# AlonKellner/hifi-gan

Hardware: NVIDIA B200
Metric: V1 audio samples/sec (higher is better)
Workload: dtype bf16

## Files before the change

hifi-gan_b200/csrc/hg_common.cuh:

```cuda
#pragma once

#include <cuda_runtime.h>
#include <cuda_bf16.h>
#include <cuda.h>
#include <stdint.h>
#include <stdio.h>

#define HG_OK 0
#define HG_ERR_INVALID (-1)
#define HG_ERR_CUDA (-2)
#define HG_ERR_UNSUPPORTED (-3)
#define HG_ERR_DRIVER (-4)

void hg_set_error(const char* fmt, ...);

#define HG_CHECK_CUDA(expr)                                                        \
  do {                                                                             \
    cudaError_t _e = (expr);                                                       \
    if (_e != cudaSuccess) {                                                       \
      hg_set_error("%s:%d: %s -> %s", __FILE__, __LINE__, #expr,                   \
                   cudaGetErrorString(_e));                                        \
      return HG_ERR_CUDA;                                                          \
    }                                                                              \
  } while (0)

#define HG_REQUIRE(cond, ...)                                                      \
  do {                                                                             \
    if (!(cond)) {                                                                 \
      hg_set_error(__VA_ARGS__);                                                   \
      return HG_ERR_INVALID;                                                       \
    }                                                                              \
  } while (0)

namespace hg {

#ifndef HG_SPIN_LIMIT
#define HG_SPIN_LIMIT (1u << 28)
#endif

__device__ __forceinline__ uint32_t smem_u32(const void* p) {
  return static_cast<uint32_t>(__cvta_generic_to_shared(p));
}

__device__ __forceinline__ bool elect_one() {
  uint32_t pred = 0;
  asm volatile(
      "{\n\t"
      ".reg .pred P;\n\t"
      "elect.sync _|P, 0xffffffff;\n\t"
      "selp.b32 %0, 1, 0, P;\n\t"
      "}\n"
      : "=r"(pred));
  return pred != 0;
}

__device__ __forceinline__ void mbar_init(uint64_t* bar, uint32_t count) {
  asm volatile("mbarrier.init.shared::cta.b64 [%0], %1;" ::"r"(smem_u32(bar)), "r"(count));
}
__device__ __forceinline__ void fence_mbar_init() {
  asm volatile("fence.mbarrier_init.release.cluster;" ::: "memory");
}
__device__ __forceinline__ void fence_proxy_async_smem() {
  asm volatile("fence.proxy.async.shared::cta;" ::: "memory");
}
__device__ __forceinline__ void mbar_arrive(uint64_t* bar) {
  asm volatile("mbarrier.arrive.shared::cta.b64 _, [%0];" ::"r"(smem_u32(bar)) : "memory");
}
__device__ __forceinline__ void mbar_arrive_expect_tx(uint64_t* bar, uint32_t bytes) {
  asm volatile("mbarrier.arrive.expect_tx.shared::cta.b64 _, [%0], %1;" ::"r"(smem_u32(bar)),
               "r"(bytes)
               : "memory");
}
__device__ __forceinline__ bool mbar_try_wait(uint64_t* bar, uint32_t parity) {
  uint32_t ok;
  asm volatile(
      "{\n\t"
      ".reg .pred P;\n\t"
      "mbarrier.try_wait.parity.shared::cta.b64 P, [%1], %2;\n\t"
      "selp.b32 %0, 1, 0, P;\n\t"
      "}\n"
      : "=r"(ok)
      : "r"(smem_u32(bar)), "r"(parity)
      : "memory");
  return ok != 0;
}
__device__ __forceinline__ void mbar_wait(uint64_t* bar, uint32_t parity) {
  uint32_t spins = 0;
  while (!mbar_try_wait(bar, parity)) {
    if (++spins > HG_SPIN_LIMIT) {
      printf("hg: mbarrier wait timed out (block %d thread %d)\n", (int)blockIdx.x, (int)threadIdx.x);
      __trap();
    }
  }
}

__device__ __forceinline__ void tma_prefetch_desc(const CUtensorMap* m) {
  asm volatile("prefetch.tensormap [%0];" ::"l"(reinterpret_cast<uint64_t>(m)) : "memory");
}
__device__ __forceinline__ void tma_load_3d(void* smem_dst, const CUtensorMap* m, uint64_t* bar,
                                            int32_t c0, int32_t c1, int32_t c2) {
  asm volatile(
      "cp.async.bulk.tensor.3d.shared::cluster.global.mbarrier::complete_tx::bytes"
      " [%0], [%1, {%3, %4, %5}], [%2];"
      :
      : "r"(smem_u32(smem_dst)), "l"(reinterpret_cast<uint64_t>(m)), "r"(smem_u32(bar)), "r"(c0),
        "r"(c1), "r"(c2)
      : "memory");
}

__device__ __forceinline__ void tc_fence_before() {
  asm volatile("tcgen05.fence::before_thread_sync;" ::: "memory");
}
__device__ __forceinline__ void tc_fence_after() {
  asm volatile("tcgen05.fence::after_thread_sync;" ::: "memory");
}
__device__ __forceinline__ void tmem_alloc(uint32_t* smem_result, uint32_t ncols) {
  asm volatile("tcgen05.alloc.cta_group::1.sync.aligned.shared::cta.b32 [%0], %1;" ::"r"(
                   smem_u32(smem_result)),
               "r"(ncols)
               : "memory");
  asm volatile("tcgen05.relinquish_alloc_permit.cta_group::1.sync.aligned;" ::: "memory");
}
__device__ __forceinline__ void tmem_dealloc(uint32_t taddr, uint32_t ncols) {
  asm volatile("tcgen05.dealloc.cta_group::1.sync.aligned.b32 %0, %1;" ::"r"(taddr), "r"(ncols)
               : "memory");
}
__device__ __forceinline__ void umma_bf16_ss_lo(uint32_t d_tmem, uint32_t a_lo, uint32_t b_lo,
                                                uint32_t desc_hi, uint32_t idesc, uint32_t accumulate) {
  asm volatile(
      "{\n\t"
      ".reg .pred p;\n\t"
      ".reg .b64 da, db;\n\t"
      "setp.ne.b32 p, %5, 0;\n\t"
      "mov.b64 da, {%1, %3};\n\t"
      "mov.b64 db, {%2, %3};\n\t"
      "tcgen05.mma.cta_group::1.kind::f16 [%0], da, db, %4, p;\n\t"
      "}\n"
      :
      : "r"(d_tmem), "r"(a_lo), "r"(b_lo), "r"(desc_hi), "r"(idesc), "r"(accumulate)
      : "memory");
}
__device__ __forceinline__ uint32_t cluster_ctarank() {
  uint32_t r;
  asm volatile("mov.u32 %0, %%cluster_ctarank;" : "=r"(r));
  return r;
}
__device__ __forceinline__ void cluster_sync_all() {
  asm volatile("barrier.cluster.arrive.release.aligned;" ::: "memory");
  asm volatile("barrier.cluster.wait.acquire.aligned;" ::: "memory");
}
__device__ __forceinline__ void mbar_arrive_remote(uint64_t* bar, uint32_t cta) {
  asm volatile(
      "{\n\t"
      ".reg .b32 remAddr32;\n\t"
      "mapa.shared::cluster.u32 remAddr32, %0, %1;\n\t"
      "mbarrier.arrive.shared::cluster.b64 _, [remAddr32];\n\t"
      "}\n"
      :
      : "r"(smem_u32(bar)), "r"(cta)
      : "memory");
}
__device__ __forceinline__ void tma_load_3d_2sm(void* smem_dst, const CUtensorMap* m, uint64_t* bar,
                                                int32_t c0, int32_t c1, int32_t c2) {
  asm volatile(
      "cp.async.bulk.tensor.3d.cta_group::2.shared::cluster.global.mbarrier::complete_tx::bytes"
      " [%0], [%1, {%3, %4, %5}], [%2];"
      :
      : "r"(smem_u32(smem_dst)), "l"(reinterpret_cast<uint64_t>(m)), "r"(smem_u32(bar) & 0xFEFFFFFFu),
        "r"(c0), "r"(c1), "r"(c2)
      : "memory");
}
__device__ __forceinline__ void tmem_alloc_2sm(uint32_t* smem_result, uint32_t ncols) {
  asm volatile("tcgen05.alloc.cta_group::2.sync.aligned.shared::cta.b32 [%0], %1;" ::"r"(
                   smem_u32(smem_result)),
               "r"(ncols)
               : "memory");
  asm volatile("tcgen05.relinquish_alloc_permit.cta_group::2.sync.aligned;" ::: "memory");
}
__device__ __forceinline__ void tmem_dealloc_2sm(uint32_t taddr, uint32_t ncols) {
  asm volatile("tcgen05.dealloc.cta_group::2.sync.aligned.b32 %0, %1;" ::"r"(taddr), "r"(ncols)
               : "memory");
}
__device__ __forceinline__ void umma_bf16_ss_lo_2sm(uint32_t d_tmem, uint32_t a_lo, uint32_t b_lo,
                                                    uint32_t desc_hi, uint32_t idesc, uint32_t accumulate) {
  asm volatile(
      "{\n\t"
      ".reg .pred p;\n\t"
      ".reg .b64 da, db;\n\t"
      "setp.ne.b32 p, %5, 0;\n\t"
      "mov.b64 da, {%1, %3};\n\t"
      "mov.b64 db, {%2, %3};\n\t"
      "tcgen05.mma.cta_group::2.kind::f16 [%0], da, db, %4, p;\n\t"
      "}\n"
      :
      : "r"(d_tmem), "r"(a_lo), "r"(b_lo), "r"(desc_hi), "r"(idesc), "r"(accumulate)
      : "memory");
}
__device__ __forceinline__ void umma_commit_2sm(uint64_t* bar) {
  asm volatile(
      "tcgen05.commit.cta_group::2.mbarrier::arrive::one.shared::cluster.multicast::cluster.b64 [%0], %1;"
      :
      : "r"(smem_u32(bar)), "h"(static_cast<uint16_t>(3))
      : "memory");
}

__device__ __forceinline__ uint32_t umma_desc_lo(uint32_t saddr) {
  return ((saddr & 0x3FFFFu) >> 4) | (1u << 16);
}
__device__ __forceinline__ uint32_t umma_desc_hi(uint32_t sbo_bytes, uint32_t layout_type) {
  return ((sbo_bytes >> 4) & 0x3FFFu) | (1u << 14) | ((layout_type & 7u) << 29);
}
__device__ __forceinline__ void umma_commit(uint64_t* bar) {
  asm volatile("tcgen05.commit.cta_group::1.mbarrier::arrive::one.shared::cluster.b64 [%0];" ::"r"(
                   smem_u32(bar))
               : "memory");
}
__device__ __forceinline__ void tmem_ld_wait() {
  asm volatile("tcgen05.wait::ld.sync.aligned;" ::: "memory");
}


__host__ __device__ constexpr uint32_t umma_idesc_bf16(uint32_t M, uint32_t N) {
  return (1u << 4) | (1u << 7) | (1u << 10) | ((N >> 3) << 17) | ((M >> 4) << 24);
}

__device__ __forceinline__ float lrelu(float v, float slope) { return v > 0.f ? v : v * slope; }

__device__ __forceinline__ uint32_t pack_bf16x2(float lo, float hi) {
  __nv_bfloat162 h = __floats2bfloat162_rn(lo, hi);
  return *reinterpret_cast<uint32_t*>(&h);
}
__device__ __forceinline__ float2 unpack_bf16x2(uint32_t w) {
  __nv_bfloat162 h = *reinterpret_cast<__nv_bfloat162*>(&w);
  return __bfloat1622float2(h);
}

struct U8 {
  uint32_t v[8];
};

__device__ __forceinline__ U8 ldg256(const void* p) {
  U8 r;
  asm volatile("ld.global.nc.L1::no_allocate.v8.b32 {%0,%1,%2,%3,%4,%5,%6,%7}, [%8];"
               : "=r"(r.v[0]), "=r"(r.v[1]), "=r"(r.v[2]), "=r"(r.v[3]), "=r"(r.v[4]), "=r"(r.v[5]),
                 "=r"(r.v[6]), "=r"(r.v[7])
               : "l"(p));
  return r;
}
__device__ __forceinline__ void stg256(void* p, const U8& r) {
  asm volatile("st.global.v8.b32 [%0], {%1,%2,%3,%4,%5,%6,%7,%8};" ::"l"(p), "r"(r.v[0]),
               "r"(r.v[1]), "r"(r.v[2]), "r"(r.v[3]), "r"(r.v[4]), "r"(r.v[5]), "r"(r.v[6]),
               "r"(r.v[7])
               : "memory");
}
__device__ __forceinline__ void tmem_ld_32x16(uint32_t taddr, uint32_t (&v)[16]) {
  asm volatile(
      "tcgen05.ld.sync.aligned.32x32b.x16.b32 "
      "{%0, %1, %2, %3, %4, %5, %6, %7, %8, %9, %10, %11, %12, %13, %14, %15}, [%16];"
      : "=r"(v[0]), "=r"(v[1]), "=r"(v[2]), "=r"(v[3]), "=r"(v[4]), "=r"(v[5]), "=r"(v[6]),
        "=r"(v[7]), "=r"(v[8]), "=r"(v[9]), "=r"(v[10]), "=r"(v[11]), "=r"(v[12]), "=r"(v[13]),
        "=r"(v[14]), "=r"(v[15])
      : "r"(taddr)
      : "memory");
}
__device__ __forceinline__ void add_bf16x16(float (&v)[16], const U8& r) {
#pragma unroll
  for (int i = 0; i < 8; ++i) {
    const float2 f = unpack_bf16x2(r.v[i]);
    v[2 * i] += f.x;
    v[2 * i + 1] += f.y;
  }
}
__device__ __forceinline__ void add_bf16x16_unlrelu(float (&v)[16], const U8& r, float inv_slope) {
#pragma unroll
  for (int i = 0; i < 8; ++i) {
    const float2 f = unpack_bf16x2(r.v[i]);
    v[2 * i] += fminf(f.x, f.x * inv_slope);
    v[2 * i + 1] += fminf(f.y, f.y * inv_slope);
  }
}



template <int N>
__device__ __forceinline__ float warp_colsum(float (&v)[N], int lane, int& col) {
  int off = 16;
  col = 0;
#pragma unroll
  for (int w = N / 2; w >= 1; w >>= 1) {
    const bool hi = (lane & off) != 0;
#pragma unroll
    for (int i = 0; i < w; ++i) {
      const float send = hi ? v[i] : v[i + w];
      const float keep = hi ? v[i + w] : v[i];
      v[i] = keep + __shfl_xor_sync(0xffffffffu, send, off);
    }
    if (hi) col += w;
    off >>= 1;
  }
#pragma unroll
  for (int o = 16; o >= 1; o >>= 1)
    if (o <= off) v[0] += __shfl_xor_sync(0xffffffffu, v[0], o);
  return v[0];
}

struct PerDeviceOnce {
  size_t done[64] = {};
  bool need(size_t want = 1) {
    int d = 0;
    if (cudaGetDevice(&d) != cudaSuccess || d < 0 || d >= 64) return true;
    if (done[d] >= want) return false;
    done[d] = want;
    return true;
  }
};
}

int hg_encode_tmap_bf16_3d(CUtensorMap* out, const void* base, uint64_t d0, uint64_t d1, uint64_t d2,
                           uint64_t stride1_bytes, uint64_t stride2_bytes, uint32_t box0,
                           uint32_t box1, uint32_t box2, int swizzle_bytes);
```

hifi-gan_b200/csrc/hg_resblock_pair.cu:

```cuda
#include "hg_common.cuh"

#include <atomic>

#include "../../include/hifigan_b200.h"

extern std::atomic<int64_t> g_hg_launches;

namespace {

constexpr int kM = 128;
constexpr int kXformWarps = 4;
__host__ __device__ constexpr int epi_halves(int c) { return c == 64 ? 2 : 1; }
__host__ __device__ constexpr int pair_threads(int c) { return 64 + (kXformWarps + 8 * epi_halves(c)) * 32; }
constexpr int kMaxXSlots = 4;

struct PairArgs {
  int batch, t, c;
  int ktaps, dil1;
  int single;
  int subs;
  int r_out;
  int pad1, pad2;
  int a_rows;
  int x_boxes, x_box_rows;
  int tiles_t, num_tiles;
  int x_slots;
  uint32_t x_slot_bytes, t1_slot_bytes, w_bytes;
  const __nv_bfloat16* x;
  const float* b1;
  const float* b2;
  const __nv_bfloat16* res1;
  const __nv_bfloat16* res2;
  float scale, in_slope, out_slope;
  __nv_bfloat16* out_raw;
  __nv_bfloat16* out_act;
  const int* item_len;
  int item_mul;
  float x_inv;
};

struct PairBarriers {
  uint64_t x_full[kMaxXSlots], x_ready[kMaxXSlots], x_empty[kMaxXSlots];
  uint64_t w_full;
  uint64_t acc1_full[2], acc1_empty[2], t1_full[2], t1_empty[2], acc2_full[2], acc2_empty[2];
  uint32_t tmem_base;
  uint32_t pad;
  __align__(16) float b1[64];
  __align__(16) float b2[64];
};

__device__ __forceinline__ uint32_t lrelu_bf16x2(uint32_t w, __nv_bfloat162 slope2) {
  __nv_bfloat162 v = *reinterpret_cast<__nv_bfloat162*>(&w);
  v = __hmax2(v, __hmul2(v, slope2));
  return *reinterpret_cast<uint32_t*>(&v);
}

template <int C, bool kSingle, bool kMrf, bool kActIn>
__global__ void __launch_bounds__(pair_threads(C), 1)
resblock_pair_kernel(const __grid_constant__ CUtensorMap tm_x, const __grid_constant__ CUtensorMap tm_w1,
                     const __grid_constant__ CUtensorMap tm_w2, const PairArgs p) {
  constexpr uint32_t kRowBytes = C * 2;
  constexpr uint32_t kLayout = (C == 64) ? 2u : 4u;
  constexpr uint32_t kSbo = 8 * kRowBytes;
  constexpr uint32_t kTapBytes = C * kRowBytes;
  constexpr int kChunksPerRow = kRowBytes / 16;
  constexpr int kHalves = epi_halves(C);
  constexpr int kRoleWarps = 4 * kHalves;
  constexpr int kThreads = pair_threads(C);

  extern __shared__ uint8_t smem_raw[];
  uint8_t* smem = reinterpret_cast<uint8_t*>((reinterpret_cast<uintptr_t>(smem_raw) + 1023) &
                                             ~static_cast<uintptr_t>(1023));
  uint8_t* x_buf = smem;
  uint8_t* t1_buf = x_buf + p.x_slots * p.x_slot_bytes;
  uint8_t* w1_buf = t1_buf + 2 * p.t1_slot_bytes;
  uint8_t* w2_buf = w1_buf + p.w_bytes;
  PairBarriers* bars = reinterpret_cast<PairBarriers*>(w1_buf + (kSingle ? 1 : 2) * p.w_bytes);

  const int warp = threadIdx.x >> 5;
  const int lane = threadIdx.x & 31;
  const int S = p.subs;
  const uint32_t acc_cols = static_cast<uint32_t>(S) * C;
  const uint32_t tmem_cols = 4 * acc_cols <= 128 ? 128u : 4 * acc_cols <= 256 ? 256u : 512u;

  if (warp == 0 && lane == 0) {
    hg::tma_prefetch_desc(&tm_x);
    hg::tma_prefetch_desc(&tm_w1);
    hg::tma_prefetch_desc(&tm_w2);
  }
  if (warp == 1) {
    if (lane == 0) {
      for (int i = 0; i < kMaxXSlots; ++i) {
        hg::mbar_init(&bars->x_full[i], 1);
        hg::mbar_init(&bars->x_ready[i], kXformWarps);
        hg::mbar_init(&bars->x_empty[i], 1);
      }
      hg::mbar_init(&bars->w_full, 1);
      for (int i = 0; i < 2; ++i) {
        hg::mbar_init(&bars->acc1_full[i], 1);
        hg::mbar_init(&bars->acc1_empty[i], kRoleWarps);
        hg::mbar_init(&bars->t1_full[i], kRoleWarps);
        hg::mbar_init(&bars->t1_empty[i], 1);
        hg::mbar_init(&bars->acc2_full[i], 1);
        hg::mbar_init(&bars->acc2_empty[i], kRoleWarps);
      }
      hg::fence_mbar_init();
    }
    __syncwarp();
    hg::tmem_alloc(&bars->tmem_base, tmem_cols);
  }
  if (threadIdx.x < C) {
    bars->b1[threadIdx.x] = p.b1[threadIdx.x];
    bars->b2[threadIdx.x] = p.b2[threadIdx.x];
  }
  for (uint32_t i = threadIdx.x * 16; i < 2 * p.t1_slot_bytes; i += kThreads * 16)
    *reinterpret_cast<uint4*>(t1_buf + i) = make_uint4(0, 0, 0, 0);
  hg::fence_proxy_async_smem();
  hg::tc_fence_before();
  __syncthreads();
  hg::tc_fence_after();
  const uint32_t tmem_base = *reinterpret_cast<volatile uint32_t*>(&bars->tmem_base);
  const int n_local = (p.num_tiles - static_cast<int>(blockIdx.x) + static_cast<int>(gridDim.x) - 1) /
                      static_cast<int>(gridDim.x);

  if (warp == 0) {
    if (lane == 0) {
      hg::mbar_arrive_expect_tx(&bars->w_full, (kSingle ? 1 : 2) * p.w_bytes);
      hg::tma_load_3d(w1_buf, &tm_w1, &bars->w_full, 0, 0, 0);
      if (!kSingle) hg::tma_load_3d(w2_buf, &tm_w2, &bars->w_full, 0, 0, 0);
      const uint32_t box_bytes = static_cast<uint32_t>(p.x_box_rows) * kRowBytes;
      int tt = blockIdx.x % p.tiles_t, b = blockIdx.x / p.tiles_t;
      const int tt_step = gridDim.x % p.tiles_t, b_step = gridDim.x / p.tiles_t;
      uint32_t slot = 0, phase = 0;
      for (int i = 0; i < n_local; ++i) {
        hg::mbar_wait(&bars->x_empty[slot], phase ^ 1u);
        hg::mbar_arrive_expect_tx(&bars->x_full[slot], box_bytes * p.x_boxes);
        for (int bx = 0; bx < p.x_boxes; ++bx)
          hg::tma_load_3d(x_buf + slot * p.x_slot_bytes + bx * box_bytes, &tm_x, &bars->x_full[slot], 0,
                          tt * p.r_out - p.pad2 - p.pad1 + bx * p.x_box_rows, b);
        if (++slot == static_cast<uint32_t>(p.x_slots)) { slot = 0; phase ^= 1u; }
        tt += tt_step; b += b_step;
        if (tt >= p.tiles_t) { tt -= p.tiles_t; ++b; }
      }
    }
    __syncwarp();
  } else if (warp == 1) {
    constexpr uint32_t idesc = hg::umma_idesc_bf16(kM, C);
    constexpr uint32_t kTapLo = kTapBytes >> 4;
    const uint32_t desc_hi = hg::umma_desc_hi(kSbo, kLayout);
    const uint32_t w1_lo = hg::umma_desc_lo(hg::smem_u32(w1_buf));
    const uint32_t w2_lo = hg::umma_desc_lo(hg::smem_u32(w2_buf));
    const uint32_t x_tap_step = static_cast<uint32_t>(p.dil1) * (kRowBytes >> 4);
    hg::mbar_wait(&bars->w_full, 0);
    hg::tc_fence_after();
    auto issue = [&](uint32_t d, uint32_t a_lo, uint32_t w_lo, uint32_t a_step) {
      uint32_t accumulate = 0;
      for (int j = 0; j < p.ktaps; ++j) {
#pragma unroll
        for (int kk = 0; kk < C / 16; ++kk) {
          hg::umma_bf16_ss_lo(d, a_lo + kk * 2, w_lo + kk * 2, desc_hi, idesc, accumulate);
          accumulate = 1;
        }
        a_lo += a_step;
        w_lo += kTapLo;
      }
    };
    uint32_t x_slot = 0, x_phase = 0;
    auto conv1 = [&](int i) {
      const uint32_t slot = x_slot, a = i & 1u, ph = (i >> 1) & 1u;
      hg::mbar_wait(&bars->x_ready[slot], x_phase);
      if (++x_slot == static_cast<uint32_t>(p.x_slots)) { x_slot = 0; x_phase ^= 1u; }
      hg::mbar_wait(&bars->acc1_empty[a], ph ^ 1u);
      hg::tc_fence_after();
      if (hg::elect_one()) {
        const uint32_t x_lo = hg::umma_desc_lo(hg::smem_u32(x_buf + slot * p.x_slot_bytes));
        for (int m = 0; m < S; ++m)
          issue(tmem_base + a * acc_cols + m * C, x_lo + m * (kM * (kRowBytes >> 4)), w1_lo, x_tap_step);
        hg::umma_commit(&bars->x_empty[slot]);
        hg::umma_commit(&bars->acc1_full[a]);
      }
      __syncwarp();
    };
    auto conv2 = [&](int i) {
      const uint32_t a = i & 1u, ph = (i >> 1) & 1u;
      hg::mbar_wait(&bars->t1_full[a], ph);
      hg::mbar_wait(&bars->acc2_empty[a], ph ^ 1u);
      hg::tc_fence_after();
      if (hg::elect_one()) {
        const uint32_t t_lo = hg::umma_desc_lo(hg::smem_u32(t1_buf + a * p.t1_slot_bytes));
        for (int m = 0; m < S; ++m)
          issue(tmem_base + 2 * acc_cols + a * acc_cols + m * C, t_lo + m * (kM * (kRowBytes >> 4)), w2_lo,
                kRowBytes >> 4);
        hg::umma_commit(&bars->t1_empty[a]);
        hg::umma_commit(&bars->acc2_full[a]);
      }
      __syncwarp();
    };
    if (kSingle) {
      for (int i = 0; i < n_local; ++i) conv1(i);
    } else {
      if (n_local > 0) conv1(0);
      for (int i = 0; i < n_local; ++i) {
        if (i + 1 < n_local) conv1(i + 1);
        conv2(i);
      }
    }
  } else if (warp < 2 + kXformWarps) {
    const int tid = (warp - 2) * 32 + lane;
    const __nv_bfloat162 slope2 = __float2bfloat162_rn(p.in_slope);
    const int n_chunks = p.a_rows * kChunksPerRow;
    uint32_t slot = 0, phase = 0;
    for (int i = 0; i < n_local; ++i) {
      hg::mbar_wait(&bars->x_full[slot], phase);
      if (!kActIn) {
        uint4* xs = reinterpret_cast<uint4*>(x_buf + slot * p.x_slot_bytes);
        for (int q = tid; q < n_chunks; q += kXformWarps * 32) {
          uint4 v = xs[q];
          v.x = lrelu_bf16x2(v.x, slope2); v.y = lrelu_bf16x2(v.y, slope2);
          v.z = lrelu_bf16x2(v.z, slope2); v.w = lrelu_bf16x2(v.w, slope2);
          xs[q] = v;
        }
        hg::fence_proxy_async_smem();
      }
      __syncwarp();
      if (lane == 0) hg::mbar_arrive(&bars->x_ready[slot]);
      if (++slot == static_cast<uint32_t>(p.x_slots)) { slot = 0; phase ^= 1u; }
    }
  } else {
    const int ew = warp - (2 + kXformWarps);
    const int quarter = warp & 3;
    const int half = (ew >> 2) % kHalves;
    const int row = quarter * 32 + lane;
    const uint32_t lane_base = static_cast<uint32_t>(quarter * 32) << 16;
    constexpr int kG = C / (16 * kHalves);
    const int col0 = half * (C / kHalves);

    if (ew < kRoleWarps) {
      const float* bias = bars->b1;
      const uint32_t swz = (C == 64) ? (row & 7) : ((row >> 1) & 3);
      int tt = blockIdx.x % p.tiles_t;
      int bb = blockIdx.x / p.tiles_t;
      const int tt_step = gridDim.x % p.tiles_t, b_step = gridDim.x / p.tiles_t;
      for (int i = 0; i < (kSingle ? 0 : n_local); ++i) {
        const uint32_t a = i & 1u, ph = (i >> 1) & 1u;
        hg::mbar_wait(&bars->acc1_full[a], ph);
        hg::mbar_wait(&bars->t1_empty[a], ph ^ 1u);
        hg::tc_fence_after();
        const int t_item = (kMrf && p.item_len) ? min(p.t, __ldg(p.item_len + bb) * p.item_mul) : p.t;
        for (int m = 0; m < S; ++m) {
          const int grow = m * kM + row;
          const int time = tt * p.r_out - p.pad2 + grow;
          const bool inside = time >= 0 && time < t_item;
          uint8_t* trow = t1_buf + a * p.t1_slot_bytes + static_cast<uint32_t>(grow) * kRowBytes;
#pragma unroll
          for (int g = 0; g < kG; ++g) {
            uint32_t raw[16];
            hg::tmem_ld_32x16(tmem_base + lane_base + a * acc_cols + m * C + col0 + g * 16, raw);
            hg::tmem_ld_wait();
            if (g == kG - 1 && m == S - 1) {
              hg::tc_fence_before();
              __syncwarp();
              if (lane == 0) hg::mbar_arrive(&bars->acc1_empty[a]);
            }
            uint32_t o[8];
#pragma unroll
            for (int q = 0; q < 4; ++q) {
              const float4 bq = *reinterpret_cast<const float4*>(bias + col0 + g * 16 + 4 * q);
              const float v0 = hg::lrelu(__uint_as_float(raw[4 * q]) + bq.x, p.in_slope);
              const float v1 = hg::lrelu(__uint_as_float(raw[4 * q + 1]) + bq.y, p.in_slope);
              const float v2 = hg::lrelu(__uint_as_float(raw[4 * q + 2]) + bq.z, p.in_slope);
              const float v3 = hg::lrelu(__uint_as_float(raw[4 * q + 3]) + bq.w, p.in_slope);
              o[2 * q] = inside ? hg::pack_bf16x2(v0, v1) : 0u;
              o[2 * q + 1] = inside ? hg::pack_bf16x2(v2, v3) : 0u;
            }
            const uint32_t chunk = (col0 >> 3) + g * 2;
            *reinterpret_cast<uint4*>(trow + ((chunk ^ swz) << 4)) = make_uint4(o[0], o[1], o[2], o[3]);
            *reinterpret_cast<uint4*>(trow + (((chunk + 1) ^ swz) << 4)) = make_uint4(o[4], o[5], o[6], o[7]);
          }
        }
        hg::fence_proxy_async_smem();
        __syncwarp();
        if (lane == 0) hg::mbar_arrive(&bars->t1_full[a]);
        tt += tt_step; bb += b_step;
        if (tt >= p.tiles_t) { tt -= p.tiles_t; ++bb; }
      }
    } else {
      const float* bias = kSingle ? bars->b1 : bars->b2;
      uint64_t* full_bar = kSingle ? bars->acc1_full : bars->acc2_full;
      uint64_t* empty_bar = kSingle ? bars->acc1_empty : bars->acc2_empty;
      const uint32_t acc_base = kSingle ? 0u : 2 * acc_cols;
      int n_tt = blockIdx.x % p.tiles_t, n_b = blockIdx.x / p.tiles_t, n_m = 0;
      const int tt_step = gridDim.x % p.tiles_t, b_step = gridDim.x / p.tiles_t;
      auto next_unit_off = [&](bool& valid, bool& keep) -> size_t {
        const int grow = n_m * kM + row;
        const int time = n_tt * p.r_out + grow;
        valid = grow < p.r_out && time < p.t;
        keep = !kMrf || !p.item_len || time < __ldg(p.item_len + n_b) * p.item_mul;
        const size_t o = (static_cast<size_t>(n_b) * p.t + (valid ? time : 0)) * C + col0;
        if (++n_m == S) {
          n_m = 0;
          n_tt += tt_step; n_b += b_step;
          if (n_tt >= p.tiles_t) { n_tt -= p.tiles_t; ++n_b; }
        }
        return o;
      };
      hg::U8 rcur[kG], rnext[kG];
      bool valid = false, valid_next = false, keep = true, keep_next = true;
      size_t off = 0, off_next = 0;
      const int n_units = n_local * S;
      if (n_units > 0) {
        off_next = next_unit_off(valid_next, keep_next);
        if (valid_next) {
#pragma unroll
          for (int g = 0; g < kG; ++g) rnext[g] = hg::ldg256(p.x + off_next + g * 16);
        }
      }
      int i = 0, m = 0;
      for (int u = 0; u < n_units; ++u) {
        const uint32_t a = i & 1u, ph = (i >> 1) & 1u;
        off = off_next; valid = valid_next; keep = keep_next;
#pragma unroll
        for (int g = 0; g < kG; ++g) rcur[g] = rnext[g];
        if (u + 1 < n_units) {
          off_next = next_unit_off(valid_next, keep_next);
          if (valid_next) {
#pragma unroll
            for (int g = 0; g < kG; ++g) rnext[g] = hg::ldg256(p.x + off_next + g * 16);
          }
        }
        constexpr bool kPreRes = kMrf && (C == 32);
        hg::U8 r1[kPreRes ? kG : 1], r2[kPreRes ? kG : 1];
        if (kPreRes && valid && p.res1) {
#pragma unroll
          for (int g = 0; g < kG; ++g) r1[kPreRes ? g : 0] = hg::ldg256(p.res1 + off + g * 16);
        }
        if (kPreRes && valid && p.res2) {
#pragma unroll
          for (int g = 0; g < kG; ++g) r2[kPreRes ? g : 0] = hg::ldg256(p.res2 + off + g * 16);
        }
        if (m == 0) {
          hg::mbar_wait(&full_bar[a], ph);
          hg::tc_fence_after();
        }
#pragma unroll
        for (int g = 0; g < kG; ++g) {
          uint32_t raw[16];
          hg::tmem_ld_32x16(tmem_base + lane_base + acc_base + a * acc_cols + m * C + col0 + g * 16, raw);
          hg::tmem_ld_wait();
          if (g == kG - 1 && m == S - 1) {
            hg::tc_fence_before();
            __syncwarp();
            if (lane == 0) hg::mbar_arrive(&empty_bar[a]);
          }
          if (valid) {
            float v[16];
#pragma unroll
            for (int q = 0; q < 4; ++q) {
              const float4 bq = *reinterpret_cast<const float4*>(bias + col0 + g * 16 + 4 * q);
              v[4 * q] = __uint_as_float(raw[4 * q]) + bq.x;
              v[4 * q + 1] = __uint_as_float(raw[4 * q + 1]) + bq.y;
              v[4 * q + 2] = __uint_as_float(raw[4 * q + 2]) + bq.z;
              v[4 * q + 3] = __uint_as_float(raw[4 * q + 3]) + bq.w;
            }
            if (kActIn) hg::add_bf16x16_unlrelu(v, rcur[g], p.x_inv);
            else hg::add_bf16x16(v, rcur[g]);
            if (kMrf && p.res1) hg::add_bf16x16(v, kPreRes ? r1[kPreRes ? g : 0] : hg::ldg256(p.res1 + off + g * 16));
            if (kMrf && p.res2) hg::add_bf16x16(v, kPreRes ? r2[kPreRes ? g : 0] : hg::ldg256(p.res2 + off + g * 16));
            if (kMrf) {
              const float sc = keep ? p.scale : 0.f;
#pragma unroll
              for (int e = 0; e < 16; ++e) v[e] *= sc;
            }
            if (p.out_raw) {
              hg::U8 o;
#pragma unroll
              for (int q = 0; q < 8; ++q) o.v[q] = hg::pack_bf16x2(v[2 * q], v[2 * q + 1]);
              hg::stg256(p.out_raw + off + g * 16, o);
            }
            if (kMrf && p.out_act) {
              hg::U8 o;
#pragma unroll
              for (int q = 0; q < 8; ++q)
                o.v[q] = hg::pack_bf16x2(hg::lrelu(v[2 * q], p.out_slope), hg::lrelu(v[2 * q + 1], p.out_slope));
              hg::stg256(p.out_act + off + g * 16, o);
            }
          }
        }
        if (++m == S) { m = 0; ++i; }
      }
    }
  }

  hg::tc_fence_before();
  __syncthreads();
  hg::tc_fence_after();
  if (warp == 1) hg::tmem_dealloc(tmem_base, tmem_cols);
}

int g_sms = 0, g_smem = 0;

template <int C, bool kSingle, bool kMrf, bool kActIn>
int launch_pair_as(const CUtensorMap& tx, const CUtensorMap& tw1, const CUtensorMap& tw2, const PairArgs& p,
                size_t smem_bytes, int grid, cudaStream_t st) {
  static hg::PerDeviceOnce once;
  if (once.need())
    HG_CHECK_CUDA(cudaFuncSetAttribute(resblock_pair_kernel<C, kSingle, kMrf, kActIn>,
                                       cudaFuncAttributeMaxDynamicSharedMemorySize, g_smem));
  resblock_pair_kernel<C, kSingle, kMrf, kActIn><<<grid, pair_threads(C), smem_bytes, st>>>(tx, tw1, tw2, p);
  HG_CHECK_CUDA(cudaGetLastError());
  return HG_OK;
}

template <int C, bool kSingle>
int launch_pair(const CUtensorMap& tx, const CUtensorMap& tw1, const CUtensorMap& tw2, const PairArgs& p,
                bool act_in, size_t smem_bytes, int grid, cudaStream_t st) {
  const bool mrf = p.res1 || p.res2 || p.out_act || p.item_len || p.scale != 1.f;
  if (act_in)
    return mrf ? launch_pair_as<C, kSingle, true, true>(tx, tw1, tw2, p, smem_bytes, grid, st)
               : launch_pair_as<C, kSingle, false, true>(tx, tw1, tw2, p, smem_bytes, grid, st);
  return mrf ? launch_pair_as<C, kSingle, true, false>(tx, tw1, tw2, p, smem_bytes, grid, st)
             : launch_pair_as<C, kSingle, false, false>(tx, tw1, tw2, p, smem_bytes, grid, st);
}

size_t pair_smem_bytes(int c, int ktaps, int dil1, int subs, int x_slots, int single, PairArgs* out) {
  const uint32_t row = static_cast<uint32_t>(c) * 2;
  const uint32_t a_rows = subs * kM + (ktaps - 1) * dil1;
  const uint32_t boxes = (a_rows + 255) / 256;
  const uint32_t box_rows = ((a_rows + boxes - 1) / boxes + 15) & ~15u;
  const uint32_t x_slot = (boxes * box_rows * row + 1023u) & ~1023u;
  const uint32_t t1_slot = single ? 0u : ((subs * kM + ktaps - 1) * row + 1023u) & ~1023u;
  const uint32_t w_bytes = static_cast<uint32_t>(ktaps) * c * row;
  if (box_rows > 256) return ~static_cast<size_t>(0);
  if (out) {
    out->subs = subs; out->a_rows = a_rows; out->x_boxes = boxes; out->x_box_rows = box_rows;
    out->x_slot_bytes = x_slot; out->t1_slot_bytes = t1_slot; out->w_bytes = w_bytes;
  }
  return 1024 + static_cast<size_t>(x_slots) * x_slot + 2 * static_cast<size_t>(t1_slot) +
         (single ? 1 : 2) * static_cast<size_t>(w_bytes) + sizeof(PairBarriers);
}

int pick_subs(int c, int ktaps, int dil1, int single) {
  for (int subs = 512 / (4 * c); subs >= 1; subs >>= 1)
    if (pair_smem_bytes(c, ktaps, dil1, subs, 2, single, nullptr) <= static_cast<size_t>(g_smem)) return subs;
  return 0;
}

}

extern "C" int hg_resblock_pair_supported(int c, int ktaps, int dil1) {
  if (!(c == 32 || c == 64) || ktaps < 1 || !(ktaps & 1) || dil1 < 1) return 0;
  if (kM + (ktaps - 1) * dil1 > 256 || ktaps > 65) return 0;
  if (!g_smem) {
    int dev = 0;
    if (cudaGetDevice(&dev) != cudaSuccess) return 0;
    cudaDeviceGetAttribute(&g_sms, cudaDevAttrMultiProcessorCount, dev);
    cudaDeviceGetAttribute(&g_smem, cudaDevAttrMaxSharedMemoryPerBlockOptin, dev);
  }
  return pick_subs(c, ktaps, dil1, 0) > 0 ? 1 : 0;
}

extern "C" int hg_resblock_single_supported(int c, int ktaps, int dil1) {
  if (!hg_resblock_pair_supported(c, 1, 1) && !g_smem) return 0;
  if (!(c == 32 || c == 64) || ktaps < 1 || !(ktaps & 1) || dil1 < 1 || ktaps > 65) return 0;
  return pick_subs(c, ktaps, dil1, 1) > 0 ? 1 : 0;
}

namespace {

int resblock_pair_fwd(const void* x, bool act_in, const void* w1_packed, const float* b1, const void* w2_packed,
                      const float* b2, int batch, int t, int c, int ktaps, int dil1, float in_slope, const void* res1,
                      const void* res2, float scale, void* out_raw, void* out_act, float out_slope,
                      const int* item_len, int item_mul, void* stream) {
  const int single = w2_packed == nullptr;
  HG_REQUIRE(x && w1_packed && b1 && (single || b2), "hg_resblock_pair_fwd: null input");
  HG_REQUIRE(out_raw || out_act, "hg_resblock_pair_fwd: no output requested");
  HG_REQUIRE(batch > 0 && t > 0, "hg_resblock_pair_fwd: empty batch/time");
  HG_REQUIRE(hg_resblock_pair_supported(c, ktaps, dil1) || (single && hg_resblock_single_supported(c, ktaps, dil1)),
             "hg_resblock_pair_fwd: unsupported shape c=%d k=%d d=%d (use hg_conv1d_fwd)", c, ktaps, dil1);
  PairArgs p{};
  p.batch = batch; p.t = t; p.c = c; p.ktaps = ktaps; p.dil1 = dil1;
  const int subs = pick_subs(c, ktaps, dil1, single);
  p.single = single;
  p.r_out = single ? subs * kM : subs * kM + 1 - ktaps;
  p.pad1 = (ktaps - 1) * dil1 / 2;
  p.pad2 = single ? 0 : (ktaps - 1) / 2;
  p.tiles_t = (t + p.r_out - 1) / p.r_out;
  p.num_tiles = batch * p.tiles_t;
  int slots = kMaxXSlots;
  while (slots > 2 && pair_smem_bytes(c, ktaps, dil1, subs, slots, single, nullptr) > static_cast<size_t>(g_smem)) --slots;
  p.x_slots = slots;
  const size_t smem_bytes = pair_smem_bytes(c, ktaps, dil1, subs, slots, single, &p);
  p.x = static_cast<const __nv_bfloat16*>(x);
  p.b1 = b1; p.b2 = single ? b1 : b2;
  p.res1 = static_cast<const __nv_bfloat16*>(res1);
  p.res2 = static_cast<const __nv_bfloat16*>(res2);
  p.scale = scale; p.in_slope = in_slope; p.out_slope = out_slope;
  p.out_raw = static_cast<__nv_bfloat16*>(out_raw);
  p.out_act = static_cast<__nv_bfloat16*>(out_act);
  p.item_len = item_len; p.item_mul = item_mul > 0 ? item_mul : 1;
  p.x_inv = act_in ? 1.f / in_slope : 1.f;

  CUtensorMap tx, tw1, tw2;
  const int swz = c * 2;
  int rc = hg_encode_tmap_bf16_3d(&tx, x, c, t, batch, static_cast<uint64_t>(c) * 2,
                                  static_cast<uint64_t>(t) * c * 2, c, p.x_box_rows, 1, swz);
  if (rc) return rc;
  rc = hg_encode_tmap_bf16_3d(&tw1, w1_packed, c, c, ktaps, static_cast<uint64_t>(c) * 2,
                              static_cast<uint64_t>(c) * c * 2, c, c, ktaps, swz);
  if (rc) return rc;
  rc = hg_encode_tmap_bf16_3d(&tw2, single ? w1_packed : w2_packed, c, c, ktaps, static_cast<uint64_t>(c) * 2,
                              static_cast<uint64_t>(c) * c * 2, c, c, ktaps, swz);
  if (rc) return rc;
  const int grid = p.num_tiles < g_sms ? p.num_tiles : g_sms;
  cudaStream_t st = static_cast<cudaStream_t>(stream);
  if (single)
    rc = (c == 64) ? launch_pair<64, true>(tx, tw1, tw2, p, act_in, smem_bytes, grid, st)
                   : launch_pair<32, true>(tx, tw1, tw2, p, act_in, smem_bytes, grid, st);
  else
    rc = (c == 64) ? launch_pair<64, false>(tx, tw1, tw2, p, act_in, smem_bytes, grid, st)
                   : launch_pair<32, false>(tx, tw1, tw2, p, act_in, smem_bytes, grid, st);
  if (rc) return rc;
  g_hg_launches.fetch_add(1, std::memory_order_relaxed);
  return HG_OK;
}

}

extern "C" int hg_resblock_pair_fwd(const void* x, const void* w1_packed, const float* b1,
                                    const void* w2_packed, const float* b2, int batch, int t, int c,
                                    int ktaps, int dil1, float in_slope, const void* res1,
                                    const void* res2, float scale, void* out_raw, void* out_act,
                                    float out_slope, const int* item_len, int item_mul, void* stream) {
  return resblock_pair_fwd(x, false, w1_packed, b1, w2_packed, b2, batch, t, c, ktaps, dil1, in_slope, res1, res2,
                           scale, out_raw, out_act, out_slope, item_len, item_mul, stream);
}

extern "C" int hg_resblock_pair_fwd_actin(const void* x_act, const void* w1_packed, const float* b1,
                                          const void* w2_packed, const float* b2, int batch, int t, int c,
                                          int ktaps, int dil1, float in_slope, const void* res1,
                                          const void* res2, float scale, void* out_raw, void* out_act,
                                          float out_slope, const int* item_len, int item_mul, void* stream) {
  HG_REQUIRE(in_slope > 0.f && in_slope <= 1.f, "hg_resblock_pair_fwd_actin: slope %g not in (0, 1]", in_slope);
  return resblock_pair_fwd(x_act, true, w1_packed, b1, w2_packed, b2, batch, t, c, ktaps, dil1, in_slope, res1, res2,
                           scale, out_raw, out_act, out_slope, item_len, item_mul, stream);
}
```

Measured before the change: 356.0 million.

## Add 2-SM cluster fused resblock pair kernel for 128-channel layers

Result: faster. 362.5 million, median of 6 (+1.8%).

```diff
diff --git a/hifi-gan_b200/csrc/hg_common.cuh b/hifi-gan_b200/csrc/hg_common.cuh
--- a/hifi-gan_b200/csrc/hg_common.cuh
+++ b/hifi-gan_b200/csrc/hg_common.cuh
@@ -160,6 +160,37 @@
       : "r"(smem_u32(bar)), "r"(cta)
       : "memory");
 }
+__device__ __forceinline__ void mbar_arrive_cluster(uint64_t* bar, uint32_t cta) {
+  asm volatile(
+      "{\n\t"
+      ".reg .b32 remAddr32;\n\t"
+      "mapa.shared::cluster.u32 remAddr32, %0, %1;\n\t"
+      "mbarrier.arrive.release.cluster.shared::cluster.b64 _, [remAddr32];\n\t"
+      "}\n"
+      :
+      : "r"(smem_u32(bar)), "r"(cta)
+      : "memory");
+}
+__device__ __forceinline__ void mbar_wait_cluster(uint64_t* bar, uint32_t parity) {
+  uint32_t spins = 0;
+  for (;;) {
+    uint32_t ok;
+    asm volatile(
+        "{\n\t"
+        ".reg .pred P;\n\t"
+        "mbarrier.try_wait.parity.acquire.cluster.shared::cta.b64 P, [%1], %2;\n\t"
+        "selp.b32 %0, 1, 0, P;\n\t"
+        "}\n"
+        : "=r"(ok)
+        : "r"(smem_u32(bar)), "r"(parity)
+        : "memory");
+    if (ok) return;
+    if (++spins > HG_SPIN_LIMIT) {
+      printf("hg: mbarrier wait timed out (block %d thread %d)\n", (int)blockIdx.x, (int)threadIdx.x);
+      __trap();
+    }
+  }
+}
 __device__ __forceinline__ void tma_load_3d_2sm(void* smem_dst, const CUtensorMap* m, uint64_t* bar,
                                                 int32_t c0, int32_t c1, int32_t c2) {
   asm volatile(
diff --git a/hifi-gan_b200/csrc/hg_resblock_pair.cu b/hifi-gan_b200/csrc/hg_resblock_pair.cu
--- a/hifi-gan_b200/csrc/hg_resblock_pair.cu
+++ b/hifi-gan_b200/csrc/hg_resblock_pair.cu
@@ -397,6 +397,330 @@
   if (warp == 1) hg::tmem_dealloc(tmem_base, tmem_cols);
 }
 
+__device__ __forceinline__ void sts128(uint32_t addr, uint32_t a, uint32_t b, uint32_t c, uint32_t d) {
+  asm volatile("st.shared.v4.b32 [%0], {%1, %2, %3, %4};" ::"r"(addr), "r"(a), "r"(b), "r"(c), "r"(d) : "memory");
+}
+
+constexpr int kPair2Threads = 64 + (kXformWarps + 16) * 32;
+constexpr int kPair2Rows = kM - 2;
+constexpr uint32_t kPair2Tap = 64 * 128;
+constexpr uint32_t kPair2WChunk = 3 * kPair2Tap;
+constexpr uint32_t kPair2T1Slab = ((kM + 2) * 128 + 1023u) & ~1023u;
+
+struct Pair2Barriers {
+  uint64_t x_full[2], x_ready[2], x_empty[2];
+  uint64_t w_full;
+  uint64_t acc1_full[2], acc1_empty[2], acc2_full[2], acc2_empty[2];
+  uint64_t t1_full, t1_empty;
+  uint32_t tmem_base;
+  uint32_t pad;
+  __align__(16) float b1[128];
+  __align__(16) float b2[128];
+};
+
+template <bool kMrf, bool kActIn>
+__global__ void __cluster_dims__(2, 1, 1) __launch_bounds__(kPair2Threads, 1)
+resblock_pair2_kernel(const __grid_constant__ CUtensorMap tm_x, const __grid_constant__ CUtensorMap tm_w1,
+                      const __grid_constant__ CUtensorMap tm_w2, const PairArgs p) {
+  constexpr uint32_t kRowBytes = 128;
+  constexpr uint32_t kSbo = 8 * kRowBytes;
+  constexpr int kRoleWarps = 8;
+  constexpr int kG = 4;
+  constexpr uint32_t kTmemCols = 512;
+
+  extern __shared__ uint8_t smem_raw[];
+  uint8_t* smem = reinterpret_cast<uint8_t*>((reinterpret_cast<uintptr_t>(smem_raw) + 1023) &
+                                             ~static_cast<uintptr_t>(1023));
+  const uint32_t x_slab = p.x_slot_bytes / 2;
+  uint8_t* x_buf = smem;
+  uint8_t* t1_buf = x_buf + 2 * p.x_slot_bytes;
+  uint8_t* w1_buf = t1_buf + 2 * kPair2T1Slab;
+  uint8_t* w2_buf = w1_buf + 2 * kPair2WChunk;
+  Pair2Barriers* bars = reinterpret_cast<Pair2Barriers*>(w2_buf + 2 * kPair2WChunk);
+
+  const int warp = threadIdx.x >> 5;
+  const int lane = threadIdx.x & 31;
+  const uint32_t rank = hg::cluster_ctarank();
+  const int n_clusters = gridDim.x >> 1;
+  const int cluster_id = blockIdx.x >> 1;
+  const int tiles_pt = (p.tiles_t + 1) >> 1;
+  const int num_pt = p.batch * tiles_pt;
+  const int n_local = cluster_id < num_pt ? (num_pt - cluster_id + n_clusters - 1) / n_clusters : 0;
+  const int ptt_step = n_clusters % tiles_pt, b_step = n_clusters / tiles_pt;
+
+  if (warp == 0 && lane == 0) {
+    hg::tma_prefetch_desc(&tm_x);
+    hg::tma_prefetch_desc(&tm_w1);
+    hg::tma_prefetch_desc(&tm_w2);
+  }
+  if (warp == 1) {
+    if (lane == 0) {
+      for (int i = 0; i < 2; ++i) {
+        hg::mbar_init(&bars->x_full[i], 1);
+        hg::mbar_init(&bars->x_ready[i], 2 * kXformWarps);
+        hg::mbar_init(&bars->x_empty[i], 1);
+        hg::mbar_init(&bars->acc1_full[i], 1);
+        hg::mbar_init(&bars->acc1_empty[i], 2 * kRoleWarps);
+        hg::mbar_init(&bars->acc2_full[i], 1);
+        hg::mbar_init(&bars->acc2_empty[i], 2 * kRoleWarps);
+      }
+      hg::mbar_init(&bars->w_full, 2);
+      hg::mbar_init(&bars->t1_full, 2 * kRoleWarps);
+      hg::mbar_init(&bars->t1_empty, 1);
+      hg::fence_mbar_init();
+    }
+    __syncwarp();
+    hg::tmem_alloc_2sm(&bars->tmem_base, kTmemCols);
+  }
+  if (threadIdx.x < 128) {
+    bars->b1[threadIdx.x] = p.b1[threadIdx.x];
+    bars->b2[threadIdx.x] = p.b2[threadIdx.x];
+  }
+  for (uint32_t i = threadIdx.x * 16; i < 2 * kPair2T1Slab; i += kPair2Threads * 16)
+    *reinterpret_cast<uint4*>(t1_buf + i) = make_uint4(0, 0, 0, 0);
+  hg::fence_proxy_async_smem();
+  hg::tc_fence_before();
+  __syncthreads();
+  hg::cluster_sync_all();
+  hg::tc_fence_after();
+  const uint32_t tmem_base = *reinterpret_cast<volatile uint32_t*>(&bars->tmem_base);
+
+  if (warp == 0) {
+    if (lane == 0) {
+      if (rank == 0) hg::mbar_arrive_expect_tx(&bars->w_full, 2 * 4 * kPair2WChunk);
+      else hg::mbar_arrive_remote(&bars->w_full, 0);
+      for (int c = 0; c < 2; ++c) {
+        hg::tma_load_3d_2sm(w1_buf + c * kPair2WChunk, &tm_w1, &bars->w_full, c * 64, static_cast<int>(rank) * 64, 0);
+        hg::tma_load_3d_2sm(w2_buf + c * kPair2WChunk, &tm_w2, &bars->w_full, c * 64, static_cast<int>(rank) * 64, 0);
+      }
+      int ptt = cluster_id % tiles_pt, b = cluster_id / tiles_pt;
+      uint32_t slot = 0, phase = 0;
+      for (int i = 0; i < n_local; ++i) {
+        const int t0 = (2 * ptt + static_cast<int>(rank)) * kPair2Rows - 1 - p.dil1;
+        hg::mbar_wait(&bars->x_empty[slot], phase ^ 1u);
+        hg::mbar_arrive_expect_tx(&bars->x_full[slot], 2 * x_slab);
+        hg::tma_load_3d(x_buf + slot * p.x_slot_bytes, &tm_x, &bars->x_full[slot], 0, t0, b);
+        hg::tma_load_3d(x_buf + slot * p.x_slot_bytes + x_slab, &tm_x, &bars->x_full[slot], 64, t0, b);
+        if (++slot == 2) { slot = 0; phase ^= 1u; }
+        ptt += ptt_step; b += b_step;
+        if (ptt >= tiles_pt) { ptt -= tiles_pt; ++b; }
+      }
+    }
+    __syncwarp();
+  } else if (warp == 1) {
+    if (rank == 0) {
+      constexpr uint32_t idesc = hg::umma_idesc_bf16(2 * kM, 128);
+      const uint32_t desc_hi = hg::umma_desc_hi(kSbo, 2u);
+      const uint32_t w1_lo = hg::umma_desc_lo(hg::smem_u32(w1_buf));
+      const uint32_t w2_lo = hg::umma_desc_lo(hg::smem_u32(w2_buf));
+      hg::mbar_wait(&bars->w_full, 0);
+      hg::tc_fence_after();
+      auto issue = [&](uint32_t d, uint32_t a_lo, uint32_t a_slab_lo, uint32_t a_step, uint32_t w_lo) {
+        uint32_t accumulate = 0;
+#pragma unroll
+        for (int j = 0; j < 3; ++j) {
+#pragma unroll
+          for (int c = 0; c < 2; ++c) {
+#pragma unroll
+            for (int kk = 0; kk < 4; ++kk) {
+              hg::umma_bf16_ss_lo_2sm(d, a_lo + c * a_slab_lo + j * a_step + kk * 2,
+                                      w_lo + c * (kPair2WChunk >> 4) + j * (kPair2Tap >> 4) + kk * 2, desc_hi, idesc,
+                                      accumulate);
+              accumulate = 1;
+            }
+          }
+        }
+      };
+      uint32_t x_slot = 0, x_phase = 0;
+      auto conv1 = [&](int i) {
+        const uint32_t slot = x_slot, a = i & 1u, ph = (i >> 1) & 1u;
+        hg::mbar_wait_cluster(&bars->x_ready[slot], x_phase);
+        if (++x_slot == 2) { x_slot = 0; x_phase ^= 1u; }
+        hg::mbar_wait(&bars->acc1_empty[a], ph ^ 1u);
+        hg::tc_fence_after();
+        if (hg::elect_one()) {
+          issue(tmem_base + a * 128, hg::umma_desc_lo(hg::smem_u32(x_buf + slot * p.x_slot_bytes)), x_slab >> 4,
+                static_cast<uint32_t>(p.dil1) * (kRowBytes >> 4), w1_lo);
+          hg::umma_commit_2sm(&bars->x_empty[slot]);
+          hg::umma_commit_2sm(&bars->acc1_full[a]);
+        }
+        __syncwarp();
+      };
+      auto conv2 = [&](int i) {
+        const uint32_t a = i & 1u, ph = (i >> 1) & 1u;
+        hg::mbar_wait_cluster(&bars->t1_full, i & 1u);
+        hg::mbar_wait(&bars->acc2_empty[a], ph ^ 1u);
+        hg::tc_fence_after();
+        if (hg::elect_one()) {
+          issue(tmem_base + 256 + a * 128, hg::umma_desc_lo(hg::smem_u32(t1_buf)), kPair2T1Slab >> 4,
+                kRowBytes >> 4, w2_lo);
+          hg::umma_commit_2sm(&bars->t1_empty);
+          hg::umma_commit_2sm(&bars->acc2_full[a]);
+        }
+        __syncwarp();
+      };
+      if (n_local > 0) conv1(0);
+      for (int i = 0; i < n_local; ++i) {
+        if (i + 1 < n_local) conv1(i + 1);
+        conv2(i);
+      }
+    }
+  } else if (warp < 2 + kXformWarps) {
+    const int tid = (warp - 2) * 32 + lane;
+    const __nv_bfloat162 slope2 = __float2bfloat162_rn(p.in_slope);
+    const int n_chunks = static_cast<int>(p.x_slot_bytes / 16);
+    uint32_t slot = 0, phase = 0;
+    for (int i = 0; i < n_local; ++i) {
+      hg::mbar_wait(&bars->x_full[slot], phase);
+      if (!kActIn) {
+        uint4* xs = reinterpret_cast<uint4*>(x_buf + slot * p.x_slot_bytes);
+        for (int q = tid; q < n_chunks; q += kXformWarps * 32) {
+          uint4 v = xs[q];
+          v.x = lrelu_bf16x2(v.x, slope2); v.y = lrelu_bf16x2(v.y, slope2);
+          v.z = lrelu_bf16x2(v.z, slope2); v.w = lrelu_bf16x2(v.w, slope2);
+          xs[q] = v;
+        }
+        hg::fence_proxy_async_smem();
+      }
+      __syncwarp();
+      if (lane == 0) hg::mbar_arrive_cluster(&bars->x_ready[slot], 0);
+      if (++slot == 2) { slot = 0; phase ^= 1u; }
+    }
+  } else {
+    const int ew = warp - (2 + kXformWarps);
+    const int quarter = warp & 3;
+    const int half = (ew >> 2) & 1;
+    const int row = quarter * 32 + lane;
+    const uint32_t lane_base = static_cast<uint32_t>(quarter * 32) << 16;
+    const int col0 = half * 64;
+    int ptt = cluster_id % tiles_pt, b = cluster_id / tiles_pt;
+
+    if (ew < kRoleWarps) {
+      const uint32_t swz = row & 7;
+      const uint32_t trow = hg::smem_u32(t1_buf) + half * kPair2T1Slab + static_cast<uint32_t>(row) * kRowBytes;
+      for (int i = 0; i < n_local; ++i) {
+        const uint32_t a = i & 1u, ph = (i >> 1) & 1u;
+        const int tt = 2 * ptt + static_cast<int>(rank);
+        const int t_item = (kMrf && p.item_len) ? min(p.t, __ldg(p.item_len + b) * p.item_mul) : p.t;
+        const int time = tt * kPair2Rows - 1 + row;
+        const bool inside = tt < p.tiles_t && time >= 0 && time < t_item;
+        hg::mbar_wait(&bars->acc1_full[a], ph);
+        hg::tc_fence_after();
+        uint32_t o[kG][8];
+        uint32_t taddr = tmem_base + lane_base + a * 128 + col0;
+#pragma unroll
+        for (int g = 0; g < kG; ++g) {
+          uint32_t raw[16];
+          hg::tmem_ld_32x16(taddr + g * 16, raw);
+          hg::tmem_ld_wait();
+#pragma unroll
+          for (int q = 0; q < 4; ++q) {
+            const float4 bq = *reinterpret_cast<const float4*>(bars->b1 + col0 + g * 16 + 4 * q);
+            const float v0 = hg::lrelu(__uint_as_float(raw[4 * q]) + bq.x, p.in_slope);
+            const float v1 = hg::lrelu(__uint_as_float(raw[4 * q + 1]) + bq.y, p.in_slope);
+            const float v2 = hg::lrelu(__uint_as_float(raw[4 * q + 2]) + bq.z, p.in_slope);
+            const float v3 = hg::lrelu(__uint_as_float(raw[4 * q + 3]) + bq.w, p.in_slope);
+            o[g][2 * q] = inside ? hg::pack_bf16x2(v0, v1) : 0u;
+            o[g][2 * q + 1] = inside ? hg::pack_bf16x2(v2, v3) : 0u;
+          }
+          asm volatile("" : "+r"(taddr) : "r"(o[g][7]));
+        }
+        hg::tc_fence_before();
+        __syncwarp();
+        if (lane == 0) {
+          if (rank == 0) hg::mbar_arrive(&bars->acc1_empty[a]);
+          else hg::mbar_arrive_remote(&bars->acc1_empty[a], 0);
+        }
+        hg::mbar_wait(&bars->t1_empty, (i & 1u) ^ 1u);
+        uint32_t tr = trow;
+        asm volatile("" : "+r"(tr));
+#pragma unroll
+        for (int g = 0; g < kG; ++g) {
+          const uint32_t chunk = g * 2;
+          sts128(tr + ((chunk ^ swz) << 4), o[g][0], o[g][1], o[g][2], o[g][3]);
+          sts128(tr + (((chunk + 1) ^ swz) << 4), o[g][4], o[g][5], o[g][6], o[g][7]);
+        }
+        hg::fence_proxy_async_smem();
+        __syncwarp();
+        if (lane == 0) hg::mbar_arrive_cluster(&bars->t1_full, 0);
+        ptt += ptt_step; b += b_step;
+        if (ptt >= tiles_pt) { ptt -= tiles_pt; ++b; }
+      }
+    } else {
+      for (int i = 0; i < n_local; ++i) {
+        const uint32_t a = i & 1u, ph = (i >> 1) & 1u;
+        const int time = (2 * ptt + static_cast<int>(rank)) * kPair2Rows + row;
+        const bool valid = row < kPair2Rows && time < p.t;
+        const bool keep = !kMrf || !p.item_len || time < __ldg(p.item_len + b) * p.item_mul;
+        const size_t off = (static_cast<size_t>(b) * p.t + (valid ? time : 0)) * 128 + col0;
+        hg::U8 rx[2];
+        if (valid) {
+          rx[0] = hg::ldg256(p.x + off);
+          rx[1] = hg::ldg256(p.x + off + 16);
+        }
+        hg::mbar_wait(&bars->acc2_full[a], ph);
+        hg::tc_fence_after();
+#pragma unroll
+        for (int g = 0; g < kG; ++g) {
+          uint32_t raw[16];
+          hg::tmem_ld_32x16(tmem_base + lane_base + 256 + a * 128 + col0 + g * 16, raw);
+          hg::tmem_ld_wait();
+          if (g == kG - 1) {
+            hg::tc_fence_before();
+            __syncwarp();
+            if (lane == 0) {
+              if (rank == 0) hg::mbar_arrive(&bars->acc2_empty[a]);
+              else hg::mbar_arrive_remote(&bars->acc2_empty[a], 0);
+            }
+          }
+          if (valid) {
+            float v[16];
+#pragma unroll
+            for (int q = 0; q < 4; ++q) {
+              const float4 bq = *reinterpret_cast<const float4*>(bars->b2 + col0 + g * 16 + 4 * q);
+              v[4 * q] = __uint_as_float(raw[4 * q]) + bq.x;
+              v[4 * q + 1] = __uint_as_float(raw[4 * q + 1]) + bq.y;
+              v[4 * q + 2] = __uint_as_float(raw[4 * q + 2]) + bq.z;
+              v[4 * q + 3] = __uint_as_float(raw[4 * q + 3]) + bq.w;
+            }
+            if (kActIn) hg::add_bf16x16_unlrelu(v, rx[g & 1], p.x_inv);
+            else hg::add_bf16x16(v, rx[g & 1]);
+            if (g + 2 < kG) rx[g & 1] = hg::ldg256(p.x + off + (g + 2) * 16);
+            if (kMrf && p.res1) hg::add_bf16x16(v, hg::ldg256(p.res1 + off + g * 16));
+            if (kMrf && p.res2) hg::add_bf16x16(v, hg::ldg256(p.res2 + off + g * 16));
+            if (kMrf) {
+              const float sc = keep ? p.scale : 0.f;
+#pragma unroll
+              for (int e = 0; e < 16; ++e) v[e] *= sc;
+            }
+            if (p.out_raw) {
+              hg::U8 o;
+#pragma unroll
+              for (int q = 0; q < 8; ++q) o.v[q] = hg::pack_bf16x2(v[2 * q], v[2 * q + 1]);
+              hg::stg256(p.out_raw + off + g * 16, o);
+            }
+            if (kMrf && p.out_act) {
+              hg::U8 o;
+#pragma unroll
+              for (int q = 0; q < 8; ++q)
+                o.v[q] = hg::pack_bf16x2(hg::lrelu(v[2 * q], p.out_slope), hg::lrelu(v[2 * q + 1], p.out_slope));
+              hg::stg256(p.out_act + off + g * 16, o);
+            }
+          }
+        }
+        ptt += ptt_step; b += b_step;
+        if (ptt >= tiles_pt) { ptt -= tiles_pt; ++b; }
+      }
+    }
+  }
+
+  hg::tc_fence_before();
+  __syncthreads();
+  hg::cluster_sync_all();
+  hg::tc_fence_after();
+  if (warp == 1) hg::tmem_dealloc_2sm(tmem_base, kTmemCols);
+}
+
 int g_sms = 0, g_smem = 0;
 
 template <int C, bool kSingle, bool kMrf, bool kActIn>
@@ -411,10 +735,34 @@
   return HG_OK;
 }
 
+bool pair_mrf(const PairArgs& p) { return p.res1 || p.res2 || p.out_act || p.item_len || p.scale != 1.f; }
+
+template <bool kMrf, bool kActIn>
+int launch_pair2_as(const CUtensorMap& tx, const CUtensorMap& tw1, const CUtensorMap& tw2, const PairArgs& p,
+                    size_t smem_bytes, int grid, cudaStream_t st) {
+  static hg::PerDeviceOnce once;
+  if (once.need())
+    HG_CHECK_CUDA(cudaFuncSetAttribute(resblock_pair2_kernel<kMrf, kActIn>,
+                                       cudaFuncAttributeMaxDynamicSharedMemorySize, g_smem));
+  resblock_pair2_kernel<kMrf, kActIn><<<grid, kPair2Threads, smem_bytes, st>>>(tx, tw1, tw2, p);
+  HG_CHECK_CUDA(cudaGetLastError());
+  return HG_OK;
+}
+
+int launch_pair2(const CUtensorMap& tx, const CUtensorMap& tw1, const CUtensorMap& tw2, const PairArgs& p,
+                 bool act_in, size_t smem_bytes, int grid, cudaStream_t st) {
+  const bool mrf = pair_mrf(p);
+  if (act_in)
+    return mrf ? launch_pair2_as<true, true>(tx, tw1, tw2, p, smem_bytes, grid, st)
+               : launch_pair2_as<false, true>(tx, tw1, tw2, p, smem_bytes, grid, st);
+  return mrf ? launch_pair2_as<true, false>(tx, tw1, tw2, p, smem_bytes, grid, st)
+             : launch_pair2_as<false, false>(tx, tw1, tw2, p, smem_bytes, grid, st);
+}
+
 template <int C, bool kSingle>
 int launch_pair(const CUtensorMap& tx, const CUtensorMap& tw1, const CUtensorMap& tw2, const PairArgs& p,
                 bool act_in, size_t smem_bytes, int grid, cudaStream_t st) {
-  const bool mrf = p.res1 || p.res2 || p.out_act || p.item_len || p.scale != 1.f;
+  const bool mrf = pair_mrf(p);
   if (act_in)
     return mrf ? launch_pair_as<C, kSingle, true, true>(tx, tw1, tw2, p, smem_bytes, grid, st)
                : launch_pair_as<C, kSingle, false, true>(tx, tw1, tw2, p, smem_bytes, grid, st);
@@ -445,10 +793,22 @@
   return 0;
 }
 
+size_t pair2_smem_bytes(int dil1, PairArgs* out) {
+  const uint32_t a_rows = kM + 2 * dil1;
+  const uint32_t box_rows = (a_rows + 7) & ~7u;
+  if (box_rows > 256) return ~static_cast<size_t>(0);
+  const uint32_t x_slot = 2 * box_rows * 128;
+  if (out) {
+    out->subs = 1; out->a_rows = a_rows; out->x_boxes = 2; out->x_box_rows = box_rows;
+    out->x_slot_bytes = x_slot; out->t1_slot_bytes = 2 * kPair2T1Slab; out->w_bytes = 4 * kPair2WChunk;
+  }
+  return 1024 + 2 * static_cast<size_t>(x_slot) + 2 * kPair2T1Slab + 2 * 2 * kPair2WChunk + sizeof(Pair2Barriers);
+}
+
 }
 
 extern "C" int hg_resblock_pair_supported(int c, int ktaps, int dil1) {
-  if (!(c == 32 || c == 64) || ktaps < 1 || !(ktaps & 1) || dil1 < 1) return 0;
+  if (!(c == 32 || c == 64 || c == 128) || ktaps < 1 || !(ktaps & 1) || dil1 < 1) return 0;
   if (kM + (ktaps - 1) * dil1 > 256 || ktaps > 65) return 0;
   if (!g_smem) {
     int dev = 0;
@@ -456,6 +816,8 @@
     cudaDeviceGetAttribute(&g_sms, cudaDevAttrMultiProcessorCount, dev);
     cudaDeviceGetAttribute(&g_smem, cudaDevAttrMaxSharedMemoryPerBlockOptin, dev);
   }
+  if (c == 128)
+    return ktaps == 3 && g_sms % 2 == 0 && pair2_smem_bytes(dil1, nullptr) <= static_cast<size_t>(g_smem) ? 1 : 0;
   return pick_subs(c, ktaps, dil1, 0) > 0 ? 1 : 0;
 }
 
@@ -475,21 +837,29 @@
   HG_REQUIRE(x && w1_packed && b1 && (single || b2), "hg_resblock_pair_fwd: null input");
   HG_REQUIRE(out_raw || out_act, "hg_resblock_pair_fwd: no output requested");
   HG_REQUIRE(batch > 0 && t > 0, "hg_resblock_pair_fwd: empty batch/time");
-  HG_REQUIRE(hg_resblock_pair_supported(c, ktaps, dil1) || (single && hg_resblock_single_supported(c, ktaps, dil1)),
+  HG_REQUIRE(single ? hg_resblock_single_supported(c, ktaps, dil1) : hg_resblock_pair_supported(c, ktaps, dil1),
              "hg_resblock_pair_fwd: unsupported shape c=%d k=%d d=%d (use hg_conv1d_fwd)", c, ktaps, dil1);
   PairArgs p{};
   p.batch = batch; p.t = t; p.c = c; p.ktaps = ktaps; p.dil1 = dil1;
-  const int subs = pick_subs(c, ktaps, dil1, single);
   p.single = single;
-  p.r_out = single ? subs * kM : subs * kM + 1 - ktaps;
   p.pad1 = (ktaps - 1) * dil1 / 2;
   p.pad2 = single ? 0 : (ktaps - 1) / 2;
+  size_t smem_bytes;
+  if (c == 128) {
+    p.r_out = kPair2Rows;
+    p.x_slots = 2;
+    smem_bytes = pair2_smem_bytes(dil1, &p);
+  } else {
+    const int subs = pick_subs(c, ktaps, dil1, single);
+    p.r_out = single ? subs * kM : subs * kM + 1 - ktaps;
+    int slots = kMaxXSlots;
+    while (slots > 2 && pair_smem_bytes(c, ktaps, dil1, subs, slots, single, nullptr) > static_cast<size_t>(g_smem))
+      --slots;
+    p.x_slots = slots;
+    smem_bytes = pair_smem_bytes(c, ktaps, dil1, subs, slots, single, &p);
+  }
   p.tiles_t = (t + p.r_out - 1) / p.r_out;
   p.num_tiles = batch * p.tiles_t;
-  int slots = kMaxXSlots;
-  while (slots > 2 && pair_smem_bytes(c, ktaps, dil1, subs, slots, single, nullptr) > static_cast<size_t>(g_smem)) --slots;
-  p.x_slots = slots;
-  const size_t smem_bytes = pair_smem_bytes(c, ktaps, dil1, subs, slots, single, &p);
   p.x = static_cast<const __nv_bfloat16*>(x);
   p.b1 = b1; p.b2 = single ? b1 : b2;
   p.res1 = static_cast<const __nv_bfloat16*>(res1);
@@ -501,18 +871,28 @@
   p.x_inv = act_in ? 1.f / in_slope : 1.f;
 
   CUtensorMap tx, tw1, tw2;
-  const int swz = c * 2;
+  const int kc = c == 128 ? 64 : c;
+  const int w_rows = c == 128 ? 64 : c;
+  const int swz = kc * 2;
   int rc = hg_encode_tmap_bf16_3d(&tx, x, c, t, batch, static_cast<uint64_t>(c) * 2,
-                                  static_cast<uint64_t>(t) * c * 2, c, p.x_box_rows, 1, swz);
+                                  static_cast<uint64_t>(t) * c * 2, kc, p.x_box_rows, 1, swz);
   if (rc) return rc;
   rc = hg_encode_tmap_bf16_3d(&tw1, w1_packed, c, c, ktaps, static_cast<uint64_t>(c) * 2,
-                              static_cast<uint64_t>(c) * c * 2, c, c, ktaps, swz);
+                              static_cast<uint64_t>(c) * c * 2, kc, w_rows, ktaps, swz);
   if (rc) return rc;
   rc = hg_encode_tmap_bf16_3d(&tw2, single ? w1_packed : w2_packed, c, c, ktaps, static_cast<uint64_t>(c) * 2,
-                              static_cast<uint64_t>(c) * c * 2, c, c, ktaps, swz);
+                              static_cast<uint64_t>(c) * c * 2, kc, w_rows, ktaps, swz);
   if (rc) return rc;
+  cudaStream_t st = static_cast<cudaStream_t>(stream);
+  if (c == 128) {
+    const int num_pt = batch * ((p.tiles_t + 1) / 2);
+    const int clusters = num_pt < g_sms / 2 ? num_pt : g_sms / 2;
+    rc = launch_pair2(tx, tw1, tw2, p, act_in, smem_bytes, 2 * clusters, st);
+    if (rc) return rc;
+    g_hg_launches.fetch_add(1, std::memory_order_relaxed);
+    return HG_OK;
+  }
   const int grid = p.num_tiles < g_sms ? p.num_tiles : g_sms;
-  cudaStream_t st = static_cast<cudaStream_t>(stream);
   if (single)
     rc = (c == 64) ? launch_pair<64, true>(tx, tw1, tw2, p, act_in, smem_bytes, grid, st)
                    : launch_pair<32, true>(tx, tw1, tw2, p, act_in, smem_bytes, grid, st);
```
